# wangchen615/kubernetes-simulator

Hardware: AMD Instinct MI355X
Metric: pod-node Filter+Score evals/sec and pods bound/sec at 50k nodes, 1-8 GPUs (higher is better)
Workload: dtype int64; 1 GPU; C3: 50k nodes w/ taints+labels, 1M-pod trace, Filter(fit+taint+selector) -> Score(LR+BA) -> argmax -> bind, 1 pod/tick; nodes=50000, trace_pods=5570560, parallelism=single-gpu, batch_pods=192

## Files before the change

kubernetes-simulator_amd/csrc/ks_engine.cpp:

```cpp
#include <cmath>
#include <numeric>
#include <cstdarg>
#include <cstdio>
#include <cstdlib>
#include <cstring>
#include <limits>

#include "ks_host.h"

using namespace ks_host;

ks_status ks_host::fail(ks_engine* e, ks_status code, const char* fmt, ...) {
    char buf[512];
    va_list ap;
    va_start(ap, fmt);
    vsnprintf(buf, sizeof buf, fmt, ap);
    va_end(ap);
    if (e) e->errmsg = buf;
    return code;
}

namespace {

constexpr int64_t kMaxNodes = 1LL << 24;
// ... 192 lines not shown
                    KS_ENGINE_CHUNK_RESOLVER | KS_ENGINE_NO_OVERLAP | KS_ENGINE_PRUNED_LISTS | KS_ENGINE_SMALL_E))
        return KS_EINVAL;
    int64_t const_total = 0, w_lr = 0, w_ba = 0;
    for (int i = 0; i < cfg->n_scorers; i++) {
        const ks_scorer& sc = cfg->scorers[i];
        if (sc.weight < 0) return KS_EINVAL;
        switch (sc.kind) {
            case KS_SCORER_CONST:
                if (sc.value < 0) return KS_EINVAL;
                const_total += (int64_t)sc.weight * sc.value;
                break;
            case KS_SCORER_LEAST_REQUESTED: w_lr += sc.weight; break;
            case KS_SCORER_BALANCED: w_ba += sc.weight; break;
            default: return KS_EINVAL;
        }
    }
    if (const_total + 10 * (w_lr + w_ba) >= (1LL << 30) - 2) return KS_EINVAL;

    ks_engine* e = new ks_engine();
    e->cfg = *cfg;
    e->device = cfg->device;
    e->B = cfg->batch_pods ? cfg->batch_pods : kDefaultBatch;
    e->flags = cfg->engine_flags;
    e->overlap = !(cfg->engine_flags & KS_ENGINE_NO_OVERLAP);
    e->dc.filter_feeds = cfg->filter_mode == KS_FILTER_FEEDS_SCORE;
    e->dc.filters = cfg->filters;
    e->dc.has_scorers = cfg->n_scorers > 0;
    e->dc.w_lr = (int32_t)w_lr;
    e->dc.w_ba = (int32_t)w_ba;
    e->dc.const_total = (int32_t)const_total;
    e->dc.tick_seconds = cfg->tick_seconds;
    *out = e;
    return KS_OK;
}

}

extern "C" {

ks_status ks_create(const ks_config* cfg, ks_engine** out) {
    ks_engine* e = nullptr;
    const ks_status v = engine_init(cfg, &e);
    if (v != KS_OK) return v;
    hipError_t r = hipSetDevice(e->device);
    if (r == hipSuccess) r = hipStreamCreateWithFlags(&e->st, hipStreamNonBlocking);
    if (r == hipSuccess) r = hipMalloc(&e->d_ctr, 32 * sizeof(int64_t));
    if (r == hipSuccess) r = hipHostMalloc(&e->h_ctr, 32 * sizeof(int64_t), hipHostMallocDefault);
    if (r == hipSuccess) r = hipMalloc(&e->d_args, sizeof(ks::EngineArgs));
    if (r == hipSuccess) r = hipHostMalloc(&e->h_args, sizeof(ks::EngineArgs), hipHostMallocDefault);
    for (int i = 0; i < 4 && r == hipSuccess; i++) r = hipEventCreate(&e->ev[i]);
    if (r == hipSuccess) r = hipMemsetAsync(e->d_ctr, 0, 32 * sizeof(int64_t), e->st);
    if (r == hipSuccess) r = hipStreamSynchronize(e->st);
    if (r != hipSuccess) {
        engine_free(e);
        return KS_EDEVICE;
    }
    *out = e;
    return KS_OK;
}

}

namespace {

void engine_free(ks_engine* e) {
    if (!e) return;
    (void)hipSetDevice(e->device);
    if (e->st) (void)hipStreamSynchronize(e->st);
    if (e->st2) (void)hipStreamSynchronize(e->st2);
    e->pods.release(); e->dur.release(); e->b_node.release(); e->b_status.release();
    e->phase_off.release(); e->cum_sec.release(); e->exp_pod.release(); e->exp_off.release();
    e->t0.release(); e->fin.release(); e->use.release(); e->expired.release(); e->exp_pos.release();
    e->preg.release(); e->d_blk.release(); e->d_digest.release(); e->srec.release();
    e->d_qs.release(); e->d_qi.release();
    if (e->node_mem) (void)hipFree(e->node_mem);
    if (e->d_ncst) (void)hipFree(e->d_ncst);
    if (e->lists) (void)hipFree(e->lists);
    if (e->cand) (void)hipFree(e->cand);
    if (e->cand_all) (void)hipFree(e->cand_all);
    if (e->lbit) (void)hipFree(e->lbit);
    if (e->lthr) (void)hipFree(e->lthr);
    if (e->comm) (void)ncclCommDestroy(e->comm);
    if (e->h_xbuf) (void)hipHostFree(e->h_xbuf);
    if (!e->group) {
        if (e->d_ctr) (void)hipFree(e->d_ctr);
        if (e->h_ctr) (void)hipHostFree(e->h_ctr);
        if (e->d_args) (void)hipFree(e->d_args);
        if (e->h_args) (void)hipHostFree(e->h_args);
    }
    if (e->d_mask) (void)hipFree(e->d_mask);
    if (e->d_score) (void)hipFree(e->d_score);
    if (e->d_sweep) (void)hipFree(e->d_sweep);
    if (e->d_eidx) (void)hipFree(e->d_eidx);
    if (e->d_nslot) (void)hipFree(e->d_nslot);
    if (e->d_first) (void)hipFree(e->d_first);
    if (e->d_spec) (void)hipFree(e->d_spec);
    if (e->d_args_spec) (void)hipFree(e->d_args_spec);
    if (e->h_args_spec) (void)hipHostFree(e->h_args_spec);
    if (e->d_args_full) (void)hipFree(e->d_args_full);
    if (e->h_args_full) (void)hipHostFree(e->h_args_full);
    if (e->pev_m) (void)hipEventDestroy(e->pev_m);
    if (e->pev_x) (void)hipEventDestroy(e->pev_x);
    if (e->st2) (void)hipStreamDestroy(e->st2);
    if (e->d_usage) (void)hipFree(e->d_usage);
    if (e->stage) (void)hipHostFree(e->stage);
    if (e->segs) (void)hipHostFree(e->segs);
    if (e->stage_ev) (void)hipEventDestroy(e->stage_ev);
    if (e->d_tick) (void)hipFree(e->d_tick);
    if (e->h_tick) (void)hipHostFree(e->h_tick);
    for (auto ev : e->ev) if (ev) (void)hipEventDestroy(ev);
    for (auto ev : e->prof_ev) (void)hipEventDestroy(ev);
    if (e->st && !e->group) (void)hipStreamDestroy(e->st);
    delete e;
}

}

extern "C" {

void ks_destroy(ks_engine* e) {
    if (e && !e->group) engine_free(e);
}

ks_status ks_comm_unique_id(uint8_t* id_out) {
    if (!id_out) return KS_EINVAL;
    ncclUniqueId uid;
    if (ncclGetUniqueId(&uid) != ncclSuccess) return KS_EDEVICE;
    static_assert(sizeof(uid) == KS_COMM_ID_BYTES, "RCCL unique id size");
    std::memcpy(id_out, &uid, sizeof uid);
    return KS_OK;
}

ks_status ks_shard(ks_engine* e, int32_t world, int32_t rank, const uint8_t* id, int32_t vshards) {
    if (!e) return KS_EINVAL;
    if (e->nodes_loaded) return fail(e, KS_EINVAL, "ks_shard must precede ks_load_nodes");
    if (e->comm) return fail(e, KS_EINVAL, "already sharded");
    if (world < 1 || rank < 0 || rank >= world || vshards < 1 || (int64_t)world * vshards > 4096)
        return fail(e, KS_EINVAL, "bad shard geometry world=%d rank=%d vshards=%d", world, rank, vshards);
    if (world > 1 && !id) return fail(e, KS_EINVAL, "world > 1 needs a communicator id");
    HIPCHK(e, hipSetDevice(e->device));
    if (id) {
        ncclUniqueId uid;
        std::memcpy(&uid, id, sizeof uid);
        const ncclResult_t r = ncclCommInitRank(&e->comm, world, uid, rank);
        if (r != ncclSuccess) {
            e->comm = nullptr;
            return fail(e, KS_EDEVICE, "ncclCommInitRank: %s", ncclGetErrorString(r));
        }
    }
    e->world = world;
    e->rank = rank;
    e->vsh = vshards;
    return KS_OK;
}

ks_status ks_shard_host(ks_engine* e, int32_t world, int32_t rank, int32_t vshards, ks_allgather_fn fn, void* user) {
    if (!e) return KS_EINVAL;
    if (e->nodes_loaded) return fail(e, KS_EINVAL, "ks_shard_host must precede ks_load_nodes");
    if (e->comm || e->xfn) return fail(e, KS_EINVAL, "already sharded");
    if (!fn || world < 1 || rank < 0 || rank >= world || vshards < 1 || (int64_t)world * vshards > 4096)
        return fail(e, KS_EINVAL, "bad host-exchange shard geometry world=%d rank=%d vshards=%d", world, rank, vshards);
    e->world = world;
    e->rank = rank;
    e->vsh = vshards;
    e->xfn = fn;
    e->xuser = user;
// ... 376 lines not shown
    for (int i = 0; i < 2 && r == hipSuccess; i++) r = hipEventCreate(&g->ev[i]);
    if (r == hipSuccess) r = hipMemsetAsync(g->d_ctr, 0, sizeof(int64_t) * 32 * max_scenarios, g->st);
    if (r == hipSuccess) r = hipStreamSynchronize(g->st);
    if (r != hipSuccess) {
        ks_group_destroy(g);
        return KS_EDEVICE;
    }
    *out = g;
    return KS_OK;
}

void ks_group_destroy(ks_group* g) {
    if (!g) return;
    (void)hipSetDevice(g->device);
    if (g->st) (void)hipStreamSynchronize(g->st);
    for (ks_engine* e : g->engs) engine_free(e);
    if (g->d_ctr) (void)hipFree(g->d_ctr);
    if (g->h_ctr) (void)hipHostFree(g->h_ctr);
    if (g->d_args) (void)hipFree(g->d_args);
    if (g->h_args) (void)hipHostFree(g->h_args);
    if (g->d_seg) (void)hipFree(g->d_seg);
    if (g->h_seg) (void)hipHostFree(g->h_seg);
    if (g->d_out) (void)hipFree(g->d_out);
    if (g->h_out) (void)hipHostFree(g->h_out);
    if (g->st2) (void)hipStreamSynchronize(g->st2);
    for (auto ev : g->ev) if (ev) (void)hipEventDestroy(ev);
    if (g->xev) (void)hipEventDestroy(g->xev);
    if (g->st2) (void)hipStreamDestroy(g->st2);
    if (g->st) (void)hipStreamDestroy(g->st);
    delete g;
}

ks_status ks_group_add(ks_group* g, const ks_config* cfg, ks_engine** out) {
    if (!g || !cfg || !out) return KS_EINVAL;
    *out = nullptr;
    if ((int)g->engs.size() >= g->cap) return KS_EINVAL;
    if (cfg->device != g->device) return KS_EINVAL;
    ks_engine* e = nullptr;
    const ks_status v = engine_init(cfg, &e);
    if (v != KS_OK) return v;
    const int idx = (int)g->engs.size();
    e->group = g;
    e->st = g->st;
    e->d_ctr = g->d_ctr + 32 * idx;
    e->h_ctr = g->h_ctr + 32 * idx;
    e->d_args = g->d_args + idx;
    e->h_args = g->h_args + idx;
    hipError_t r = hipSetDevice(g->device);
    for (int i = 0; i < 4 && r == hipSuccess; i++) r = hipEventCreate(&e->ev[i]);
    if (r != hipSuccess) {
        engine_free(e);
        return KS_EDEVICE;
    }
    g->engs.push_back(e);
    *out = e;
    return KS_OK;
}

int32_t ks_group_size(const ks_group* g) { return g ? (int32_t)g->engs.size() : -1; }


int64_t ks_current_tick(const ks_engine* e) { return e ? e->tick : -1; }
int32_t ks_tick_seconds(const ks_engine* e) { return e ? e->cfg.tick_seconds : -1; }
int64_t ks_queued_pods(const ks_engine* e) { return e ? e->P - e->done : -1; }
const char* ks_last_error(const ks_engine* e) { return e ? e->errmsg.c_str() : "null engine"; }

ks_status ks_last_step_stats(const ks_engine* e, ks_step_stats* out) {
    if (!e || !out) return KS_EINVAL;
    *out = e->stats;
    return KS_OK;
}

ks_status ks_last_step_kernels(const ks_engine* e, ks_kernel_stats* out) {
    if (!e || !out) return KS_EINVAL;
    *out = e->kstats;
    return KS_OK;
}

ks_status ks_debug_counters(ks_engine* e, int64_t* out32) {
    if (!e || !out32) return KS_EINVAL;
    HIPCHK(e, hipSetDevice(e->device));
    HIPCHK(e, hipMemcpyAsync(out32, e->d_ctr, 32 * sizeof(int64_t), hipMemcpyDeviceToHost, e->st));
    HIPCHK(e, hipStreamSynchronize(e->st));
    return KS_OK;
}

#ifndef KS_SRC_HASH
#define KS_SRC_HASH "unhashed"
#endif
const char* ks_build_id(void) { return KS_SRC_HASH; }

ks_status ks_debug_invariants(ks_engine* e, int64_t* out4) {
    if (!e || !out4) return KS_EINVAL;
    out4[0] = out4[1] = out4[2] = out4[3] = 0;
    if (!e->d_sweep) return KS_OK;
    HIPCHK(e, hipSetDevice(e->device));
    std::vector<int32_t> ns(e->n_pad), ei(e->n_pad), fi(e->n_pad);
    int32_t hw = 0;
    HIPCHK(e, hipMemcpyAsync(ns.data(), e->d_nslot, sizeof(int32_t) * e->n_pad, hipMemcpyDeviceToHost, e->st));
    HIPCHK(e, hipMemcpyAsync(fi.data(), e->d_first, sizeof(int32_t) * e->n_pad, hipMemcpyDeviceToHost, e->st));
    HIPCHK(e, hipMemcpyAsync(ei.data(), e->d_eidx, sizeof(int32_t) * e->n_pad, hipMemcpyDeviceToHost, e->st));
    HIPCHK(e, hipMemcpyAsync(&hw, &e->d_sweep->nslot_hw, sizeof hw, hipMemcpyDeviceToHost, e->st));
    HIPCHK(e, hipStreamSynchronize(e->st));
    for (int64_t i = 0; i < e->n_pad; i++) {
        out4[0] += ns[i] != -1 || fi[i] != ks::kNoFirst;
        out4[1] += ei[i] != -1;
    }
    out4[2] = hw;
    out4[3] = ks::kSlotMax;
    return KS_OK;
}

ks_status ks_debug_window(ks_engine* e, void* out, int64_t cap, int64_t* size_out) {
    if (!e || !size_out) return KS_EINVAL;
    *size_out = (int64_t)sizeof(ks::WinWS);
    if (!e->d_sweep || !out || cap <= 0) return KS_OK;
    HIPCHK(e, hipSetDevice(e->device));
    HIPCHK(e, hipMemcpyAsync(out, e->d_sweep, std::min<int64_t>(cap, sizeof(ks::WinWS)), hipMemcpyDeviceToHost, e->st));
    HIPCHK(e, hipStreamSynchronize(e->st));
    return KS_OK;
}

ks_status ks_debug_watch(ks_engine* e, int64_t pod) {
    if (!e) return KS_EINVAL;
#ifdef KS_BATCH_LOG
    if (ks_status r = ensure_window_ws(e); r != KS_OK) return r;
    const int32_t w[2] = {(int32_t)pod, 0};
    HIPCHK(e, hipSetDevice(e->device));
    HIPCHK(e, hipMemcpyAsync(&e->d_sweep->watch_pod, w, sizeof w, hipMemcpyHostToDevice, e->st));
    HIPCHK(e, hipStreamSynchronize(e->st));
    return KS_OK;
#else
    (void)pod;
    return KS_EINVAL;
#endif
}

void ks_set_profiling(ks_engine* e, int enable) {
    if (e) e->profiling = enable != 0;
}
}
```

kubernetes-simulator_amd/csrc/ks_host.h:

```cpp
#pragma once
#include <hip/hip_runtime.h>
#include <rccl/rccl.h>

#include <algorithm>
#include <functional>
#include <queue>
#include <string>
#include <unordered_map>
#include <vector>

#include "../../include/ks_engine.h"
#include "ks_device.h"
#include "ks_plan.h"

namespace ks_host {

constexpr int64_t kMaxValue = 1LL << 59;
constexpr int kDefaultBatch = 256;
constexpr int64_t kUBlk = 256;
constexpr int64_t kUSup = 64;
constexpr int64_t kMaxDigestTicks = 1 << 20;

template <typename T>
struct DVec {
// ... 47 lines not shown
};

}

struct ks_engine {
    template <typename T>
    using DVec = ks_host::DVec<T>;
    ks_config cfg{};
    ks::Cfg dc{};
    hipStream_t st = nullptr;
    int device = 0;
    bool profiling = false;

    int64_t n = 0, n_pad = 0;
    int nwb = 0;
    bool nodes_loaded = false;
    void* node_mem = nullptr;
    uint4* d_ncst = nullptr;
    ks::NodeSoA s{};

    DVec<ks::PodRec> pods;
    DVec<int32_t> dur, b_node, b_status, phase_off, cum_sec, exp_pod;
    DVec<int64_t> exp_off, t0, fin, use, exp_pos;
    DVec<uint8_t> expired;
    DVec<ks::ScanRec> srec;
    std::vector<int64_t> h_bind_tick, h_fin;
    std::vector<int64_t> h_exp_off{0};
    std::vector<int32_t> h_dur;
    std::vector<int32_t> h_total_sec;
    ks_host::PendingHeap pending;
    int64_t P = 0, F = 0;
    int64_t last_arrival = 0;
    int64_t scale[3] = {1, 1, 1};
    int64_t max_alloc[3] = {0, 0, 0};
    int mode = ks::kEvalWide;
    uint32_t flags = 0;
    std::vector<int64_t> h_exp_pos;
    std::vector<int64_t> h_key;
    std::unordered_map<int64_t, int64_t> key_end;
    std::vector<int32_t> h_node;
    std::vector<int8_t> h_status;
    std::vector<ks::PodRec> h_pods;
    std::vector<int32_t> h_exp_pod;
    std::vector<uint8_t> h_expired;
    uint8_t* stage = nullptr;
    uint8_t* stage_dev = nullptr;
    int64_t stage_cap = 0, stage_used = 0;
    ks::CopySeg* segs = nullptr;
    ks::CopySeg* segs_dev = nullptr;
    int seg_cap = 0, nseg = 0, seg_done = 0;
    int64_t xpos_lo = INT64_MAX;
    hipEvent_t stage_ev = nullptr;
    ks::TickScratch* d_tick = nullptr;
    ks::TickOut* h_tick = nullptr;
    ks::TickOut* h_tick_dev = nullptr;
    int64_t idx_upto = 0;
    std::vector<std::vector<int64_t>> node_pods;
    std::vector<int64_t> h_end, blk_end, sup_end;
    DVec<uint8_t> preg;

    int64_t tick = 0, done = 0;
    int err = KS_OK;
    std::string errmsg;

    int B = ks_host::kDefaultBatch, PG = 32;
    uint64_t* lists = nullptr;
    uint64_t* cand = nullptr;
    int nblk = 0;
    int world = 1, rank = 0, vsh = 1;
    ncclComm_t comm = nullptr;
    ks_allgather_fn xfn = nullptr;
    void* xuser = nullptr;
    uint64_t* h_xbuf = nullptr;
    std::vector<int> part_lo;
    int blk_lo = 0, blk_n = 0;
    uint64_t* cand_all = nullptr;
    bool prune = false;
    int L = ks::kTopL;
    uint64_t* lbit = nullptr;
    uint64_t* lthr = nullptr;
    int nwl = 0;
    int64_t* d_ctr = nullptr;
    int64_t* h_ctr = nullptr;
    ks::EngineArgs* d_args = nullptr;
    ks::EngineArgs* h_args = nullptr;
    bool overlap = true;
    int scan_workers = 0;
    int64_t* d_spec = nullptr;
    ks::EngineArgs* d_args_spec = nullptr;
    ks::EngineArgs* h_args_spec = nullptr;
    hipStream_t st2 = nullptr;
    hipEvent_t pev_m = nullptr, pev_x = nullptr;
    ks::EngineArgs* d_args_full = nullptr;
    ks::EngineArgs* h_args_full = nullptr;
    ks_group* group = nullptr;
    hipEvent_t ev[4] = {nullptr, nullptr, nullptr, nullptr};
    std::vector<hipEvent_t> prof_ev;
    ks_step_stats stats{};
    ks_kernel_stats kstats{};

    uint8_t* d_mask = nullptr;
    int64_t* d_score = nullptr;
    ks::WinWS* d_sweep = nullptr;
    int32_t* d_eidx = nullptr;
    int32_t* d_nslot = nullptr;
    int32_t* d_first = nullptr;
    unsigned long long* d_usage = nullptr;
    DVec<int32_t> d_blk;
    std::vector<int32_t> h_blk;
    DVec<unsigned long long> d_digest;
    std::vector<int64_t> h_arr;
    std::vector<int64_t> cum_ok{0}, cum_over{0};
    int64_t cum_upto = 0;
    DVec<unsigned long long> d_qs;
    DVec<int32_t> d_qi;
    std::vector<ks::PodRec> h_shapes;
};

namespace ks_host {

enum { kEvStepBegin = 0, kEvStepEnd = 1, kEvUsageBegin = 2, kEvUsageEnd = 3 };

ks_status fail(ks_engine* e, ks_status code, const char* fmt, ...);

#define HIPCHK(e, expr)                                                                              \
    do {                                                                                             \
        hipError_t _r = (expr);                                                                      \
        if (_r != hipSuccess)                                                                        \
            return ks_host::fail((e), KS_EDEVICE, "%s failed: %s", #expr, hipGetErrorString(_r));    \
    } while (0)

hipError_t stage_flush(ks_engine* e);
hipError_t stage_xpos(ks_engine* e);
ks::EngineArgs make_args(ks_engine* e);
bool in_passed_domain(const ks_engine* e, int64_t first_bind, int64_t t);
bool key16(const ks_engine* e);
bool small_resolver(const ks_engine* e);
int resolver_of(const ks_engine* e);
hipError_t launch_resolver(const ks::EngineArgs* d, int S, int mode, int which, hipStream_t st);
ks_status ensure_window_ws(ks_engine* e);
ks_status flush_expiries(ks_engine* e);

}

struct ks_group {
    int device = 0;
    int cap = 0;
    hipStream_t st = nullptr;
    std::vector<ks_engine*> engs;
    int64_t* d_ctr = nullptr;
    int64_t* h_ctr = nullptr;
    ks::EngineArgs* d_args = nullptr;
    ks::EngineArgs* h_args = nullptr;
    ks::BindSeg* d_seg = nullptr;
    ks::BindSeg* h_seg = nullptr;
    int32_t* d_out = nullptr;
    int32_t* h_out = nullptr;
    int64_t out_cap = 0;
    hipEvent_t ev[2] = {nullptr, nullptr};
    hipStream_t st2 = nullptr;
    hipEvent_t xev = nullptr;
    std::string errmsg;
};
```

kubernetes-simulator_amd/csrc/ks_plan.h:

```cpp
#pragma once
#include <stdint.h>

#include "../../include/ks_engine.h"
#include "ks_device.h"

namespace ks_host {

#ifndef KS_OVERLAP_MAX_BLOCKS
#define KS_OVERLAP_MAX_BLOCKS 256
#endif
constexpr int kOverlapMaxBlocks = KS_OVERLAP_MAX_BLOCKS;

enum Resolver { kResolveRole = 0, kResolveSmall = 1, kResolveChunk = 4 };

enum Chain { kChainPlain, kChainOverlapSharded, kChainTwoLaunch, kChainPipe };

struct StepPlan {
    int resolver;
    Chain chain;
    int L;
};

struct PlanFacts {
    int resolver;
    bool overlap;
    bool spec_args;
    bool key16;
    int blk_n;
    int parts;
    bool prune;
    bool side_stream;
};

inline StepPlan plan_step(const PlanFacts& f) {
    const bool fused = f.resolver == kResolveChunk;
    const bool overlap = fused && f.overlap && f.spec_args && f.key16 && f.blk_n <= kOverlapMaxBlocks;
    const bool pipe = fused && !overlap && f.overlap && f.side_stream && f.parts > 1;
    StepPlan p{f.resolver, kChainPlain, ks::kTopL};
    if (pipe) p.chain = kChainPipe;
    else if (overlap) p.chain = f.parts == 1 ? kChainTwoLaunch : kChainOverlapSharded;
    if ((p.chain == kChainTwoLaunch && !f.prune) || p.chain == kChainPipe) p.L = ks::kTopLOverlap;
    return p;
}

enum Mark {
    kMarkBegin,
    kMarkPrep,
    kMarkScan,
    kMarkParts,
    kMarkXchg,
    kMarkMerge,
    kMarkResolve,
    kMarkSideBegin,
    kMarkSideScan,
    kMarkSideParts,
    kMarkSideXchg,
    kMarkCount
};

struct BatchRecord {
    Chain chain;
    bool prep_launched;
    bool scan_launched;
    bool fused;
    bool sharded;
    uint32_t recorded;
};

inline BatchRecord batch_record(Chain chain, bool first, bool more, bool sharded) {
    switch (chain) {
        case kChainPlain: return BatchRecord{chain, true, true, false, sharded, 0};
        case kChainOverlapSharded: return BatchRecord{chain, first, true, more, true, 0};
        case kChainTwoLaunch: return BatchRecord{chain, first, first, more, false, 0};
        default: return BatchRecord{chain, first, true, more, true, 0};
    }
}

enum Interval {
    kIvPrep,
    kIvScan,
    kIvParts,
    kIvXchg,
    kIvMergeTail,
    kIvMergeAll,
    kIvResolve,
    kIvSideScan,
    kIvSideParts,
    kIvSideXchg,
    kIvCount
};
constexpr Mark kIntervalEnds[kIvCount][2] = {
    {kMarkBegin, kMarkPrep},        {kMarkPrep, kMarkScan},          {kMarkScan, kMarkParts},
    {kMarkParts, kMarkXchg},        {kMarkXchg, kMarkMerge},         {kMarkScan, kMarkMerge},
    {kMarkMerge, kMarkResolve},     {kMarkSideBegin, kMarkSideScan}, {kMarkSideScan, kMarkSideParts},
    {kMarkSideParts, kMarkSideXchg}};
inline bool interval_recorded(const BatchRecord& r, int iv) {
    return (r.recorded >> kIntervalEnds[iv][0] & 1) && (r.recorded >> kIntervalEnds[iv][1] & 1);
}

struct StepSums {
    double scan_ms = 0, resolve_ms = 0, other_ms = 0;
};

inline void account_batch(const BatchRecord& r, const float* t, ks_kernel_stats& ks, StepSums& s) {
    const float rs = t[kIvResolve];
    if (r.chain == kChainPipe) {
        const float w = t[kIvPrep], sc = t[kIvScan], pm = t[kIvParts], xc = t[kIvXchg], mg = t[kIvMergeTail];
        ks.wait_ms += w;
        ks.scan_ms += sc; ks.scan_n += 1; s.scan_ms += sc;
        ks.merge_ms += pm + xc + mg; ks.merge_n += 1; s.other_ms += pm + xc + mg + w;
        if (r.prep_launched) { ks.part_ms += pm; ks.xchg_ms += xc; ks.xchg_n += 1; }
        if (r.fused) {
            ks.side_scan_ms += t[kIvSideScan]; ks.side_part_ms += t[kIvSideParts]; ks.side_xchg_ms += t[kIvSideXchg];
            ks.side_n += 1;
        }
    } else {
        if (r.sharded) { ks.part_ms += t[kIvParts]; ks.xchg_ms += t[kIvXchg]; ks.xchg_n += 1; }
        s.other_ms += t[kIvPrep] + t[kIvMergeAll];
        s.scan_ms += t[kIvScan];
        ks.prep_ms += t[kIvPrep]; ks.prep_n += r.prep_launched ? 1 : 0;
        ks.scan_ms += t[kIvScan]; ks.scan_n += r.scan_launched ? 1 : 0;
        ks.merge_ms += t[kIvMergeAll]; ks.merge_n += 1;
    }
    if (r.fused) { ks.fused_ms += rs; ks.fused_n += 1; }
    else { ks.resolve_ms += rs; ks.resolve_n += 1; }
// ... 5 lines not shown
```

kubernetes-simulator_amd/csrc/ks_step.cpp:

```cpp
#include <cstdlib>
#include <cstring>
#include <thread>

#include "ks_host.h"

using namespace ks_host;

namespace {

constexpr int kRescanWgs = 1024;

bool step_prepare(ks_engine* e, int64_t ticks, int64_t* p_hi_out) {
    const int64_t t_end = e->tick + ticks;
    const int64_t p_hi = std::upper_bound(e->h_bind_tick.begin() + e->done, e->h_bind_tick.end(), t_end) -
                         e->h_bind_tick.begin();
    *p_hi_out = p_hi;
    e->stats = ks_step_stats{};
    e->kstats = ks_kernel_stats{};
    e->h_ctr[0] = e->done;
    e->h_ctr[1] = std::max(p_hi, e->done);
    e->h_ctr[2] = 0;
    e->h_ctr[3] = -1;
    e->h_ctr[4] = 0;
    *e->h_args = make_args(e);
    return p_hi > e->done;
}

ks_status device_stop(ks_engine* e, ks_status r) {
    if (r == KS_EDEVICE && e->err == KS_OK) {
        e->err = KS_EDEVICE;
        if (e->errmsg.empty()) e->errmsg = "device failure during a step";
    }
    return r;
}

ks_status step_finish(ks_engine* e, int64_t t_end, int64_t new_done, const int32_t* node, const int32_t* status,
                      ks_bind* out, int64_t cap, int64_t* n_out) {
    const int64_t nb = new_done - e->done;
    for (int64_t i = 0; i < nb && i < cap; i++) {
        out[i].pod = e->done + i;
        out[i].node = node[i];
        out[i].status = status[i];
        out[i].tick = e->h_bind_tick[e->done + i];
    }
    for (int64_t i = 0; i < nb; i++) {
        e->h_node[e->done + i] = node[i];
        e->h_status[e->done + i] = (int8_t)status[i];
    }
    *n_out = nb;
    e->done = new_done;
    if (e->h_ctr[2] != 0) {
        const int64_t pod = e->h_ctr[3];
        e->err = (int)e->h_ctr[2];
        e->tick = e->h_bind_tick[pod];
        e->done = pod + 1;
        if (e->err == KS_ENOTFOUND)
            fail(e, KS_ENOTFOUND, "node \"\" not found (pod %lld, tick %lld)", (long long)pod, (long long)e->tick);
        else
            fail(e, KS_EINVAL, "pod %lld: invalid pod key or simSpec (tick %lld)", (long long)pod, (long long)e->tick);
        return (ks_status)e->err;
    }
    e->tick = t_end;
    return KS_OK;
}

void mirror_expired(ks_engine* e, int64_t lo, int64_t hi) {
    for (int64_t j = lo; j < hi; j++)
        for (int64_t u = e->h_exp_off[j]; u < e->h_exp_off[j + 1]; u++) {
            const int32_t q = e->h_exp_pod[u];
            if (e->h_status[q] == KS_POD_OK) e->h_expired[q] = 1;
        }
}

bool tick_step(ks_engine* e, int64_t t_end, ks_bind* out, int64_t cap, int64_t* n_out, ks_status* rc) {
    const int64_t j = e->done;
    ks::TickArgs a{};
    for (int64_t u = e->h_exp_off[j]; u < e->h_exp_off[j + 1]; u++) {
        const int32_t q = e->h_exp_pod[u];
        if (e->h_status[q] != KS_POD_OK || e->h_expired[q]) continue;
        if (a.n_exp == ks::kTickMaxExp) return false;
        ks::TickExp& x = a.exp[a.n_exp++];
        x.node = e->h_node[q];
        x.q = q;
        for (int k = 0; k < 3; k++) x.req[k] = e->h_pods[q].req[k];
    }
    *rc = KS_OK;
    if (!e->d_tick) {
        hipError_t r = hipMalloc(&e->d_tick, sizeof(ks::TickScratch));
        if (r == hipSuccess) r = hipMemsetAsync(e->d_tick, 0, sizeof(ks::TickScratch), e->st);
        if (r == hipSuccess) r = hipHostMalloc(&e->h_tick, sizeof(ks::TickOut), hipHostMallocMapped);
        if (r == hipSuccess) r = hipHostGetDevicePointer((void**)&e->h_tick_dev, e->h_tick, 0);
        if (r == hipSuccess && !e->stage_ev) r = hipEventCreateWithFlags(&e->stage_ev, hipEventDisableTiming);
        if (r != hipSuccess) { *rc = fail(e, KS_EDEVICE, "per-tick path setup: %s", hipGetErrorString(r)); return true; }
    }
    a.c = e->dc;
    a.s = e->s;
    a.pod = e->h_pods[j];
    a.j = j;
    a.run = e->h_dur[j] > 0;
    a.b_node = e->b_node.p;
    a.b_status = e->b_status.p;
    a.expired = e->expired.p;
    a.scr = e->d_tick;
    a.out = e->h_tick_dev;
    if (stage_xpos(e) != hipSuccess) { *rc = fail(e, KS_EDEVICE, "per-tick path: staging failed"); return true; }
    {
        int32_t off = 0;
        bool fits = e->nseg - e->seg_done <= ks::kTickInlSeg;
        for (int k = e->seg_done; fits && k < e->nseg; k++) {
            off += (int32_t)((e->segs[k].bytes + 15) / 16 * 16);
            fits = off <= ks::kTickInl;
        }
        if (fits) {
            off = 0;
            for (int k = e->seg_done; k < e->nseg; k++) {
                const ks::CopySeg& sg = e->segs[k];
                std::memcpy(a.inl + off, e->stage + (sg.src - e->stage_dev), (size_t)sg.bytes);
                a.iseg[a.n_iseg++] = ks::TickSeg{sg.dst, off, (int32_t)sg.bytes};
                off += (int32_t)((sg.bytes + 15) / 16 * 16);
            }
            e->seg_done = e->nseg;
        } else if (stage_flush(e) != hipSuccess) {
            *rc = fail(e, KS_EDEVICE, "per-tick path: staging failed");
            return true;
        }
    }
    __atomic_store_n(&e->h_tick->code, -1, __ATOMIC_RELAXED);
    hipError_t r = ks::launch_tick(a, e->mode, e->st);
    if (r == hipSuccess) r = hipEventRecord(e->stage_ev, e->st);
    for (uint32_t spin = 1; r == hipSuccess; spin++) {
        if (__atomic_load_n(&e->h_tick->code, __ATOMIC_ACQUIRE) >= 0) break;
        if ((spin & 1023) == 0) {
            const hipError_t q = hipStreamQuery(e->st);
            if (q == hipSuccess) break;
            if (q != hipErrorNotReady) r = q;
        }
        __builtin_ia32_pause();
    }
    if (r != hipSuccess) { *rc = fail(e, KS_EDEVICE, "per-tick launch: %s", hipGetErrorString(r)); return true; }
    ks::TickOut o;
    o.code = __atomic_load_n(&e->h_tick->code, __ATOMIC_ACQUIRE);
    o.node = ((volatile ks::TickOut*)e->h_tick)->node;
    o.status = ((volatile ks::TickOut*)e->h_tick)->status;
    for (int k = 0; k < a.n_exp; k++) e->h_expired[a.exp[k].q] = 1;
    e->stats = ks_step_stats{};
    e->stats.launches = 1;
// ... 227 lines not shown
    HIPCHK(e, pf.mark(kMarkMerge, st));
    HIPCHK(e, chunk_resolve(e, pos, e->scan_workers, e->L));
    HIPCHK(e, pf.mark(kMarkResolve, st));
    return KS_OK;
}

ks_status batch_pipe(ks_engine* e, const BatchPos& pos, StepProfile& pf) {
    hipStream_t st = e->st, s2 = e->st2;
    const ks::EngineArgs* d = e->d_args;
    HIPCHK(e, pf.begin(kChainPipe, pos, true));
    HIPCHK(e, pf.mark(kMarkBegin, st));
    if (pos.first) {
        HIPCHK(e, ks::launch_window_prep(d, true, false, (int)(pos.b & 1), st));
        HIPCHK(e, pf.mark(kMarkPrep, st));
        ks::ScanOpts so = scan_opts(e);
        so.stage = true;
        HIPCHK(e, scan(e, d, e->blk_n, st, so));
        HIPCHK(e, pf.mark(kMarkScan, st));
        if (ks_status r = parts_and_exchange(e, pf, d, st, -1, kMarkParts, kMarkXchg); r != KS_OK) return r;
    } else {
        HIPCHK(e, hipStreamWaitEvent(st, e->pev_x, 0));
        HIPCHK(e, pf.mark(kMarkPrep, st));
        ks::ScanOpts rescan = scan_opts(e);
        rescan.cond = true;
        rescan.stage = true;
        rescan.pw = kRescanWgs;
        HIPCHK(e, scan(e, e->d_args_full, e->nblk, st, rescan));
        HIPCHK(e, pf.mark(kMarkScan, st));
        HIPCHK(e, pf.mark(kMarkParts, st));
        HIPCHK(e, pf.mark(kMarkXchg, st));
    }
    ks::MergeClOpts mo;
    mo.L = e->L;
    mo.own_fallback = !pos.first;
    HIPCHK(e, ks::launch_merge_cl(d, e->mode, e->B, ks::exchanged_lists(e->cand_all, e->world * e->vsh, e->B, e->L), st, mo));
    HIPCHK(e, pf.mark(kMarkMerge, st));
    if (pos.more) HIPCHK(e, hipEventRecord(e->pev_m, st));
    HIPCHK(e, chunk_resolve(e, pos, 0, ks::kTopL));
    HIPCHK(e, pf.mark(kMarkResolve, st));
    if (pos.more) {
        const ks::EngineArgs* ds = e->d_args_spec + (pos.b & 1);
        HIPCHK(e, hipStreamWaitEvent(s2, e->pev_m, 0));
        HIPCHK(e, pf.mark(kMarkSideBegin, s2));
        HIPCHK(e, scan(e, ds, e->blk_n, s2, scan_opts(e)));
        HIPCHK(e, pf.mark(kMarkSideScan, s2));
        if (ks_status r = parts_and_exchange(e, pf, ds, s2, 0, kMarkSideParts, kMarkSideXchg); r != KS_OK) return r;
        HIPCHK(e, hipEventRecord(e->pev_x, s2));
    }
    return KS_OK;
}

ks_status chain_batch(ks_engine* e, const StepPlan& plan, const BatchPos& pos, StepProfile& pf) {
    switch (plan.chain) {
        case kChainOverlapSharded: return batch_overlap_sharded(e, pos, pf);
        case kChainTwoLaunch: return batch_two_launch(e, pos, pf);
        case kChainPipe: return batch_pipe(e, pos, pf);
        default: return batch_plain(e, plan, pos, pf);
    }
}

ks_status upload_args(ks_engine* e, const StepPlan& plan) {
    hipStream_t st = e->st;
    const bool two = plan.chain == kChainTwoLaunch;
    e->h_args->two_launch = two ? 1 : 0;
    HIPCHK(e, hipMemcpyAsync(e->d_args, e->h_args, sizeof(ks::EngineArgs), hipMemcpyHostToDevice, st));
    if (two) HIPCHK(e, ks::launch_node_consts(e->s, e->n_pad, e->d_ncst, st));
    if (plan.chain == kChainPipe) {
        *e->h_args_full = *e->h_args;
        e->h_args_full->blk_lo = 0;
        e->h_args_full->blk_n = e->nblk;
        HIPCHK(e, hipMemcpyAsync(e->d_args_full, e->h_args_full, sizeof(ks::EngineArgs), hipMemcpyHostToDevice, st));
    }
    if (plan.chain != kChainPlain) {
        for (int k = 0; k < 2; k++) {
            e->h_args_spec[k] = *e->h_args;
            e->h_args_spec[k].ctr = e->d_spec + ks::kSpecStride * k;
            e->h_args_spec[k].lset = 0;
        }
        HIPCHK(e, hipMemcpyAsync(e->d_args_spec, e->h_args_spec, 2 * sizeof(ks::EngineArgs), hipMemcpyHostToDevice, st));
    }
    return KS_OK;
}

ks_status step_body(ks_engine* e, int64_t ticks, ks_bind* out, int64_t cap, int64_t* n_out) {
    HIPCHK(e, hipSetDevice(e->device));
    if (ks_status r = ensure_window_ws(e); r != KS_OK) return r;
    const int64_t t_end = e->tick + ticks;
    int64_t p_hi = 0;
    if (!step_prepare(e, ticks, &p_hi)) {
        e->tick = t_end;
        return KS_OK;
    }
    if (p_hi == e->done + 1 && !e->group && e->world * e->vsh == 1 && e->n > 0 && !e->profiling &&
        !(e->flags & (KS_ENGINE_CHUNK_RESOLVER | KS_ENGINE_ONE_POD_RESOLVER))) {
        ks_status rc = KS_OK;
        if (tick_step(e, t_end, out, cap, n_out, &rc)) return rc;
    }
    const int64_t done0 = e->done;
    HIPCHK(e, stage_flush(e));
    hipStream_t st = e->st;
    PlanFacts facts{};
    facts.resolver = resolver_of(e);
    facts.overlap = e->overlap;
    facts.spec_args = e->d_args_spec != nullptr;
    facts.key16 = key16(e);
    facts.blk_n = e->blk_n;
    facts.parts = e->world * e->vsh;
    facts.prune = e->prune;
    facts.side_stream = e->st2 != nullptr;
    const StepPlan plan = plan_step(facts);
    e->L = plan.L;
    HIPCHK(e, hipMemcpyAsync(e->d_ctr, e->h_ctr, 5 * sizeof(int64_t), hipMemcpyHostToDevice, st));
    if (ks_status r = upload_args(e, plan); r != KS_OK) return r;
    HIPCHK(e, hipEventRecord(e->ev[kEvStepBegin], st));
    int64_t start = e->done;
    int64_t launches = 0;
    StepProfile pf{e, {}};
    while (true) {
        const int64_t nbat = (p_hi - start + e->B - 1) / e->B;
        for (int64_t b = 0; b < nbat; b++, launches++)
            if (ks_status r = chain_batch(e, plan, BatchPos{b, b == 0, b + 1 < nbat}, pf); r != KS_OK) return r;
        HIPCHK(e, hipMemcpyAsync(e->h_ctr, e->d_ctr, 5 * sizeof(int64_t), hipMemcpyDeviceToHost, st));
        HIPCHK(e, hipStreamSynchronize(st));
        const int64_t prev = start;
        start = e->h_ctr[0];
        if (e->h_ctr[2] != 0 || start >= p_hi) break;
        if (start <= prev) return fail(e, KS_EDEVICE, "scheduling made no progress at pod %lld", (long long)start);
    }
    HIPCHK(e, hipEventRecord(e->ev[kEvStepEnd], st));
    const int64_t new_done = start;
    const int64_t nb = new_done - e->done;
    std::vector<int32_t> node(nb), status(nb);
    if (nb) {
        HIPCHK(e, hipMemcpyAsync(node.data(), e->b_node.p + e->done, sizeof(int32_t) * nb, hipMemcpyDeviceToHost, st));
        HIPCHK(e, hipMemcpyAsync(status.data(), e->b_status.p + e->done, sizeof(int32_t) * nb, hipMemcpyDeviceToHost, st));
    }
    HIPCHK(e, hipStreamSynchronize(st));
    float ms = 0;
    (void)hipEventElapsedTime(&ms, e->ev[kEvStepBegin], e->ev[kEvStepEnd]);
    ks_kernel_stats ks{};
    StepSums sums;
    pf.account(ks, sums);
    e->kstats = ks;
    e->stats.step_ms = ms;
    e->stats.scan_ms = sums.scan_ms;
    e->stats.resolve_ms = sums.resolve_ms;
    e->stats.other_ms = sums.other_ms;
    e->stats.launches = launches;
    e->stats.pods = nb;
    const ks_status rc = step_finish(e, t_end, new_done, node.data(), status.data(), out, cap, n_out);
    if (rc == KS_OK) mirror_expired(e, done0, e->done);
    return rc;
}

}

extern "C" {

ks_status ks_step(ks_engine* e, int64_t ticks, ks_bind* out, int64_t cap, int64_t* n_out) {
    if (!e || !n_out || ticks < 0 || cap < 0 || (cap > 0 && !out)) return KS_EINVAL;
    *n_out = 0;
    if (e->err) return (ks_status)e->err;
    if (!e->nodes_loaded) return fail(e, KS_EINVAL, "no nodes loaded");
    if (e->P > 0 && !in_passed_domain(e, e->h_bind_tick[0], e->tick + ticks))
        return fail(e, KS_ERANGE, "step to tick %lld: more than 2^31 s after the first bind (tick %lld)",
                    (long long)(e->tick + ticks), (long long)e->h_bind_tick[0]);
    return device_stop(e, step_body(e, ticks, out, cap, n_out));
}

#ifndef KS_GROUP_SPLIT_MIN
#define KS_GROUP_SPLIT_MIN 64
#endif
constexpr int kGroupSplitMin = KS_GROUP_SPLIT_MIN;

ks_status ks_group_step(ks_group* g, int64_t ticks, ks_bind* out, int64_t cap, int64_t* n_out, int32_t* status_out,
                        ks_step_stats* stats) {
    if (!g || !n_out || !status_out || ticks < 0 || cap < 0) return KS_EINVAL;
    const int S = (int)g->engs.size();
    if (S == 0) return KS_OK;
    if (hipSetDevice(g->device) != hipSuccess) return KS_EDEVICE;
    std::vector<int64_t> p_hi(S, 0), t_end(S, 0);
    std::vector<char> live(S, 0), part(S, 0);
    int mode = ks::kEvalMicro, blk_n = 0, B = 0;
    bool k16 = true, small = true;
    for (ks_engine* e : g->engs) {
        B = std::max(B, e->B);
        k16 = k16 && key16(e);
        small = small && small_resolver(e);
    }
    const int which = small ? kResolveSmall : kResolveRole;
    int64_t blocks = 0;
    for (int i = 0; i < S; i++) {
        ks_engine* e = g->engs[i];
        n_out[i] = 0;
        status_out[i] = KS_OK;
        const bool out_of_domain = e->P > 0 && !in_passed_domain(e, e->h_bind_tick[0], e->tick + ticks);
        if (e->err || !e->nodes_loaded || e->world * e->vsh != 1 || out_of_domain) {
            status_out[i] = e->err ? e->err : out_of_domain ? KS_ERANGE : KS_EINVAL;
            if (!e->err) {
                if (out_of_domain) fail(e, KS_ERANGE, "step past 2^31 s after the first bind");
                else fail(e, KS_EINVAL, "group step needs loaded, unsharded nodes");
            }
            e->h_ctr[0] = e->h_ctr[1] = e->done;
            e->h_ctr[2] = 0;
            *e->h_args = e->nodes_loaded ? make_args(e) : ks::EngineArgs{};
            e->h_args->ctr = e->d_ctr;
            e->h_args->blk_n = 0;
            continue;
        }
        t_end[i] = e->tick + ticks;
        part[i] = 1;
        live[i] = step_prepare(e, ticks, &p_hi[i]);
        mode = std::min(mode, e->mode);
        blk_n = std::max(blk_n, e->blk_n);
        blocks += e->blk_n;
    }
    int pg = 1;
    while (pg < ks::max_pods_per_scan_wg() && pg < B && blocks * ((B + pg * 2 - 1) / (pg * 2)) >= 2048) pg *= 2;
    for (int i = 0; i < S; i++) g->h_args[i].PG = pg;
    hipStream_t st = g->st;
    auto dev = [&](hipError_t r) { return r == hipSuccess; };
    auto dev_fail = [&](const char* what) {
        g->errmsg = what;
        for (int i = 0; i < S; i++)
            if (part[i]) {
                ks_engine* e = g->engs[i];
                e->err = KS_EDEVICE;
                e->errmsg = what;
                status_out[i] = KS_EDEVICE;
            }
        return KS_EDEVICE;
    };
    if (!dev(hipMemcpyAsync(g->d_ctr, g->h_ctr, sizeof(int64_t) * 32 * S, hipMemcpyHostToDevice, st)) ||
        !dev(hipMemcpyAsync(g->d_args, g->h_args, sizeof(ks::EngineArgs) * S, hipMemcpyHostToDevice, st)) ||
// ... 108 lines not shown
```

Before: 99.68 billion evals/s.

## Overlap bind readback and host row processing with tail GPU rounds

Replaces the per-step std::vector allocation and post-sync copy of bind results with persistent pinned host buffers. A counter snapshot is taken a few rounds before the end; pods already finished by then are copied on a side stream and processed on the host (bind rows, expired mirror) while the remaining GPU rounds run. When little work remains, the tail copy is enqueued on the main stream before the sync. This is meant to hide readback and host post-processing latency behind GPU work, at the cost of an extra event sync, more complex bookkeeping, and the risk of mismatched ranges if the loop repeats.

After: 101.1 billion evals/s, median of 6. +1.4%, better.

```diff
diff --git a/kubernetes-simulator_amd/csrc/ks_engine.cpp b/kubernetes-simulator_amd/csrc/ks_engine.cpp
--- a/kubernetes-simulator_amd/csrc/ks_engine.cpp
+++ b/kubernetes-simulator_amd/csrc/ks_engine.cpp
@@ -298,6 +298,10 @@
     if (e->lthr) (void)hipFree(e->lthr);
     if (e->comm) (void)ncclCommDestroy(e->comm);
     if (e->h_xbuf) (void)hipHostFree(e->h_xbuf);
+    if (e->st_copy) { (void)hipStreamSynchronize(e->st_copy); (void)hipStreamDestroy(e->st_copy); }
+    if (e->snap_ev) (void)hipEventDestroy(e->snap_ev);
+    if (e->h_bnode) (void)hipHostFree(e->h_bnode);
+    if (e->h_bstat) (void)hipHostFree(e->h_bstat);
     if (!e->group) {
         if (e->d_ctr) (void)hipFree(e->d_ctr);
         if (e->h_ctr) (void)hipHostFree(e->h_ctr);
@@ -840,6 +844,10 @@
     HIPCHK(e, hipSetDevice(e->device));
     HIPCHK(e, hipMemcpyAsync(out32, e->d_ctr, 32 * sizeof(int64_t), hipMemcpyDeviceToHost, e->st));
     HIPCHK(e, hipStreamSynchronize(e->st));
+#if !defined(KS_CHUNK_DIAG) && !defined(KS_MCL_DIAG)
+    out32[8] = e->early_pods;
+    out32[9] = e->snap_pods;
+#endif
     return KS_OK;
 }
 
diff --git a/kubernetes-simulator_amd/csrc/ks_host.h b/kubernetes-simulator_amd/csrc/ks_host.h
--- a/kubernetes-simulator_amd/csrc/ks_host.h
+++ b/kubernetes-simulator_amd/csrc/ks_host.h
@@ -153,6 +153,12 @@
     int nwl = 0;
     int64_t* d_ctr = nullptr;
     int64_t* h_ctr = nullptr;
+    int32_t* h_bnode = nullptr;
+    int32_t* h_bstat = nullptr;
+    int64_t bind_cap = 0;
+    hipStream_t st_copy = nullptr;
+    hipEvent_t snap_ev = nullptr;
+    int64_t early_pods = 0, snap_pods = 0;
     ks::EngineArgs* d_args = nullptr;
     ks::EngineArgs* h_args = nullptr;
     bool overlap = true;
diff --git a/kubernetes-simulator_amd/csrc/ks_plan.h b/kubernetes-simulator_amd/csrc/ks_plan.h
--- a/kubernetes-simulator_amd/csrc/ks_plan.h
+++ b/kubernetes-simulator_amd/csrc/ks_plan.h
@@ -41,6 +41,15 @@
     else if (overlap) p.chain = f.parts == 1 ? kChainTwoLaunch : kChainOverlapSharded;
     if ((p.chain == kChainTwoLaunch && !f.prune) || p.chain == kChainPipe) p.L = ks::kTopLOverlap;
     return p;
+}
+
+#ifndef KS_EARLY_READBACK
+#define KS_EARLY_READBACK 1
+#endif
+constexpr int kEarlyMinRounds = 16;
+constexpr int kEarlyK = 6;
+inline int64_t early_round(int64_t rounds, Chain chain) {
+    return KS_EARLY_READBACK && chain == kChainTwoLaunch && rounds >= kEarlyMinRounds ? rounds - 1 - kEarlyK : -1;
 }
 
 enum Mark {
diff --git a/kubernetes-simulator_amd/csrc/ks_step.cpp b/kubernetes-simulator_amd/csrc/ks_step.cpp
--- a/kubernetes-simulator_amd/csrc/ks_step.cpp
+++ b/kubernetes-simulator_amd/csrc/ks_step.cpp
@@ -1,3 +1,4 @@
+#include <algorithm>
 #include <cstdlib>
 #include <cstring>
 #include <thread>
@@ -9,6 +10,7 @@
 namespace {
 
 constexpr int kRescanWgs = 1024;
+constexpr int64_t kCopyBehindMax = 4096;
 
 bool step_prepare(ks_engine* e, int64_t ticks, int64_t* p_hi_out) {
     const int64_t t_end = e->tick + ticks;
@@ -34,20 +36,24 @@
     return r;
 }
 
-ks_status step_finish(ks_engine* e, int64_t t_end, int64_t new_done, const int32_t* node, const int32_t* status,
-                      ks_bind* out, int64_t cap, int64_t* n_out) {
-    const int64_t nb = new_done - e->done;
-    for (int64_t i = 0; i < nb && i < cap; i++) {
-        out[i].pod = e->done + i;
-        out[i].node = node[i];
-        out[i].status = status[i];
-        out[i].tick = e->h_bind_tick[e->done + i];
-    }
-    for (int64_t i = 0; i < nb; i++) {
-        e->h_node[e->done + i] = node[i];
-        e->h_status[e->done + i] = (int8_t)status[i];
-    }
-    *n_out = nb;
+void bind_rows(ks_engine* e, int64_t lo, int64_t hi, const int32_t* node, const int32_t* status, ks_bind* out,
+               int64_t cap) {
+    const int64_t base = e->done;
+    for (int64_t j = lo; j < hi && j - base < cap; j++) {
+        ks_bind& o = out[j - base];
+        o.pod = j;
+        o.node = node[j - base];
+        o.status = status[j - base];
+        o.tick = e->h_bind_tick[j];
+    }
+    for (int64_t j = lo; j < hi; j++) {
+        e->h_node[j] = node[j - base];
+        e->h_status[j] = (int8_t)status[j - base];
+    }
+}
+
+ks_status step_close(ks_engine* e, int64_t t_end, int64_t new_done, int64_t* n_out) {
+    *n_out = new_done - e->done;
     e->done = new_done;
     if (e->h_ctr[2] != 0) {
         const int64_t pod = e->h_ctr[3];
@@ -62,6 +68,12 @@
     }
     e->tick = t_end;
     return KS_OK;
+}
+
+ks_status step_finish(ks_engine* e, int64_t t_end, int64_t new_done, const int32_t* node, const int32_t* status,
+                      ks_bind* out, int64_t cap, int64_t* n_out) {
+    bind_rows(e, e->done, new_done, node, status, out, cap);
+    return step_close(e, t_end, new_done, n_out);
 }
 
 void mirror_expired(ks_engine* e, int64_t lo, int64_t hi) {
@@ -455,7 +467,64 @@
     return KS_OK;
 }
 
+ks_status ensure_readback(ks_engine* e, int64_t n, bool early) {
+    if (n > e->bind_cap) {
+        const int64_t want = std::max<int64_t>({n, 2 * e->bind_cap, 4096});
+        if (e->h_bnode) (void)hipHostFree(e->h_bnode);
+        if (e->h_bstat) (void)hipHostFree(e->h_bstat);
+        e->h_bnode = e->h_bstat = nullptr;
+        e->bind_cap = 0;
+        HIPCHK(e, hipHostMalloc(&e->h_bnode, sizeof(int32_t) * want, hipHostMallocDefault));
+        HIPCHK(e, hipHostMalloc(&e->h_bstat, sizeof(int32_t) * want, hipHostMallocDefault));
+        e->bind_cap = want;
+    }
+    if (early && !e->st_copy) {
+        HIPCHK(e, hipStreamCreateWithFlags(&e->st_copy, hipStreamNonBlocking));
+        HIPCHK(e, hipEventCreateWithFlags(&e->snap_ev, hipEventDisableTiming));
+    }
+    return KS_OK;
+}
+
+ks_status copy_binds(ks_engine* e, int64_t done0, int64_t lo, int64_t hi, hipStream_t s) {
+    if (hi <= lo) return KS_OK;
+    const size_t bytes = sizeof(int32_t) * (size_t)(hi - lo);
+    HIPCHK(e, hipMemcpyAsync(e->h_bnode + (lo - done0), e->b_node.p + lo, bytes, hipMemcpyDeviceToHost, s));
+    HIPCHK(e, hipMemcpyAsync(e->h_bstat + (lo - done0), e->b_status.p + lo, bytes, hipMemcpyDeviceToHost, s));
+    return KS_OK;
+}
+
+#ifdef KS_TAIL_SPLIT
+}
+#include <chrono>
+#include <cstdio>
+namespace {
+enum { kTsPrepare, kTsUpload, kTsEnqueue, kTsSnapWait, kTsEarlyCopy, kTsEarlyRows, kTsEarlyMirror, kTsSync, kTsStats,
+       kTsRows, kTsMirror, kTsCount };
+constexpr const char* kTsNames[kTsCount] = {"prepare", "upload", "enqueue", "snap_wait", "early_copy", "early_rows",
+                                            "early_mirror", "sync", "stats", "rows", "mirror"};
+#define TAIL_BEGIN()                                               \
+    double tail_us[kTsCount] = {};                                 \
+    auto tail_t = std::chrono::steady_clock::now()
+#define TAIL_AT(I)                                                                             \
+    do {                                                                                       \
+        const auto t_ = std::chrono::steady_clock::now();                                      \
+        tail_us[I] += std::chrono::duration<double, std::micro>(t_ - tail_t).count();          \
+        tail_t = t_;                                                                           \
+    } while (0)
+#define TAIL_PRINT()                                                                           \
+    do {                                                                                       \
+        std::fprintf(stderr, "tail_split");                                                    \
+        for (int i_ = 0; i_ < kTsCount; i_++) std::fprintf(stderr, " %s=%.1f", kTsNames[i_], tail_us[i_]); \
+        std::fprintf(stderr, "\n");                                                            \
+    } while (0)
+#else
+#define TAIL_BEGIN()
+#define TAIL_AT(I)
+#define TAIL_PRINT()
+#endif
+
 ks_status step_body(ks_engine* e, int64_t ticks, ks_bind* out, int64_t cap, int64_t* n_out) {
+    TAIL_BEGIN();
     HIPCHK(e, hipSetDevice(e->device));
     if (ks_status r = ensure_window_ws(e); r != KS_OK) return r;
     const int64_t t_end = e->tick + ticks;
@@ -483,32 +552,76 @@
     facts.side_stream = e->st2 != nullptr;
     const StepPlan plan = plan_step(facts);
     e->L = plan.L;
+    if (ks_status r = ensure_readback(e, p_hi - done0, plan.chain == kChainTwoLaunch); r != KS_OK) return r;
+    TAIL_AT(kTsPrepare);
     HIPCHK(e, hipMemcpyAsync(e->d_ctr, e->h_ctr, 5 * sizeof(int64_t), hipMemcpyHostToDevice, st));
     if (ks_status r = upload_args(e, plan); r != KS_OK) return r;
+    TAIL_AT(kTsUpload);
     HIPCHK(e, hipEventRecord(e->ev[kEvStepBegin], st));
-    int64_t start = e->done;
+    int64_t start = done0;
     int64_t launches = 0;
+    int64_t have = done0, fin = done0, snap_pods = 0;
+    const int32_t* const node = e->h_bnode;
+    const int32_t* const status = e->h_bstat;
     StepProfile pf{e, {}};
     while (true) {
-        const int64_t nbat = (p_hi - start + e->B - 1) / e->B;
-        for (int64_t b = 0; b < nbat; b++, launches++)
-            if (ks_status r = chain_batch(e, plan, BatchPos{b, b == 0, b + 1 < nbat}, pf); r != KS_OK) return r;
+        const int64_t rounds = (p_hi - start + e->B - 1) / e->B;
+        const int64_t snap_at = early_round(rounds, plan.chain);
+        for (int64_t b = 0; b < rounds; b++, launches++) {
+            if (ks_status r = chain_batch(e, plan, BatchPos{b, b == 0, b + 1 < rounds}, pf); r != KS_OK) return r;
+            if (b == snap_at) {
+                HIPCHK(e, hipMemcpyAsync(e->h_ctr + 8, e->d_ctr + ks::kCtrStart, sizeof(int64_t), hipMemcpyDeviceToHost, st));
+                HIPCHK(e, hipEventRecord(e->snap_ev, st));
+            }
+        }
+        HIPCHK(e, hipEventRecord(e->ev[kEvStepEnd], st));
         HIPCHK(e, hipMemcpyAsync(e->h_ctr, e->d_ctr, 5 * sizeof(int64_t), hipMemcpyDeviceToHost, st));
+        TAIL_AT(kTsEnqueue);
+        if (fin < have) {
+            bind_rows(e, fin, have, node, status, out, cap);
+            mirror_expired(e, fin, have);
+            fin = have;
+            TAIL_AT(kTsEarlyMirror);
+        }
+        int64_t lo = start;
+        const bool snapped = snap_at >= 0 && have == start;
+        if (snapped) {
+            HIPCHK(e, hipEventSynchronize(e->snap_ev));
+            TAIL_AT(kTsSnapWait);
+            lo = std::clamp(e->h_ctr[8], start, p_hi);
+        }
+        const bool behind = have == start && p_hi - lo <= kCopyBehindMax;
+        if (behind)
+            if (ks_status r = copy_binds(e, done0, lo, p_hi, st); r != KS_OK) return r;
+        if (snapped && lo > have) {
+            if (ks_status r = copy_binds(e, done0, have, lo, e->st_copy); r != KS_OK) return r;
+            HIPCHK(e, hipStreamSynchronize(e->st_copy));
+            snap_pods += lo - have;
+            have = lo;
+            TAIL_AT(kTsEarlyCopy);
+            bind_rows(e, fin, have, node, status, out, cap);
+            TAIL_AT(kTsEarlyRows);
+            mirror_expired(e, fin, have);
+            TAIL_AT(kTsEarlyMirror);
+            fin = have;
+        }
         HIPCHK(e, hipStreamSynchronize(st));
+        TAIL_AT(kTsSync);
         const int64_t prev = start;
         start = e->h_ctr[0];
+        if (behind) have = std::clamp(start, have, p_hi);
         if (e->h_ctr[2] != 0 || start >= p_hi) break;
         if (start <= prev) return fail(e, KS_EDEVICE, "scheduling made no progress at pod %lld", (long long)start);
     }
-    HIPCHK(e, hipEventRecord(e->ev[kEvStepEnd], st));
+    if (have < start) {
+        if (ks_status r = copy_binds(e, done0, have, start, st); r != KS_OK) return r;
+        HIPCHK(e, hipStreamSynchronize(st));
+        TAIL_AT(kTsSync);
+    }
     const int64_t new_done = start;
-    const int64_t nb = new_done - e->done;
-    std::vector<int32_t> node(nb), status(nb);
-    if (nb) {
-        HIPCHK(e, hipMemcpyAsync(node.data(), e->b_node.p + e->done, sizeof(int32_t) * nb, hipMemcpyDeviceToHost, st));
-        HIPCHK(e, hipMemcpyAsync(status.data(), e->b_status.p + e->done, sizeof(int32_t) * nb, hipMemcpyDeviceToHost, st));
-    }
-    HIPCHK(e, hipStreamSynchronize(st));
+    const int64_t nb = new_done - done0;
+    e->early_pods = fin - done0;
+    e->snap_pods = snap_pods;
     float ms = 0;
     (void)hipEventElapsedTime(&ms, e->ev[kEvStepBegin], e->ev[kEvStepEnd]);
     ks_kernel_stats ks{};
@@ -521,8 +634,13 @@
     e->stats.other_ms = sums.other_ms;
     e->stats.launches = launches;
     e->stats.pods = nb;
-    const ks_status rc = step_finish(e, t_end, new_done, node.data(), status.data(), out, cap, n_out);
-    if (rc == KS_OK) mirror_expired(e, done0, e->done);
+    TAIL_AT(kTsStats);
+    bind_rows(e, std::min(fin, new_done), new_done, node, status, out, cap);
+    TAIL_AT(kTsRows);
+    const ks_status rc = step_close(e, t_end, new_done, n_out);
+    if (rc == KS_OK) mirror_expired(e, std::min(fin, new_done), new_done);
+    TAIL_AT(kTsMirror);
+    TAIL_PRINT();
     return rc;
 }
 
```
